# drprojects/DeepViewAgg

Hardware: AMD Instinct MI355X
Metric: points/sec fused fwd+bwd (1M pts, 32 views) (higher is better)
Workload: dtype bf16

## Files before the change

### deepviewagg_amd/csrc/chain_bwd.hip

```cpp
#include "chain_common.h"

namespace dva {
namespace chain {

struct ChainKeep {
  f32x16 z5, z6, t6;
  bf16x8 a2[2], a5[2], a6[2];
};
template <int W6F, int L6, bool MASK = true>
__device__ __forceinline__ void chain_forward(const uint4* s_ops, int lane, const float (*tabs)[TAB_FLOATS], int h,
                                              uint32_t keep, const float4& x, const f32x16& uacc, ChainKeep& k) {
  const f32x16 zero = {0};
  bf16x8 a1[2];
  asm volatile("" ::: "memory");
  const f32x16 t1 = CH_MFMA(lds_op(s_ops, OP_W1, lane), pack_x(x), bias_acc(tabs[0], T_B6, h));
  act_fold<MASK>(t1, keep, a1);
  const f32x16 t2 = mm32_lds(s_ops, OP_W2, lane, a1, bias_acc(tabs[1], T_B6, h));
  act_fold<MASK>(t2, keep, k.a2);
  k.z5 = mm32_lds(s_ops, OP_W5, lane, k.a2, uacc);
  act_pack<MASK>(k.z5, tabs[2], h, keep, k.a5);
  k.z6 = mm32_lds(s_ops, OP_W6, lane, k.a5, zero);
  if (L6 >= 1) k.t6 = mm32_lds(s_ops, W6F, lane, k.a5, bias_acc(tabs[3], T_B6, h));
  if (L6 >= 2) act_fold<MASK>(k.t6, keep, k.a6);
}
// ... 321 lines not shown
    const float* __restrict__ bn1, const float* __restrict__ bn2, const float* __restrict__ bn5,
    const float* __restrict__ bn6, const float* __restrict__ dc, double* __restrict__ stats6,
    float* __restrict__ dWs, float* __restrict__ dbs, int G, int64_t V, int64_t N, const float* __restrict__ qp,
    float qscale) {
  constexpr int L_W6F = 7, L_WST = 9, NOPS = KEYS ? 11 : 10;
  __shared__ __attribute__((aligned(16))) float s_tab[4][TAB_FLOATS];
  __shared__ __attribute__((aligned(16))) uint4 s_ops[NOPS * 64];
  __shared__ __attribute__((aligned(16))) bf16_t s_tc[4][32 * TSB], s_td[4][(KEYS ? 32 : 5) * TSB];
  float* s_red = reinterpret_cast<float*>(&s_tc[0][0]);
  static_assert(sizeof(bf16_t) * 4 * 32 * TSB >= sizeof(float) * D * D, "epilogue buffer");
  const int lane = threadIdx.x & 63, wv = threadIdx.x >> 6, j = lane & 31, h = lane >> 5;
  for (int i = threadIdx.x; i < 4 * (KEYS ? 32 : 5) * TSB; i += blockDim.x) (&s_td[0][0])[i] = 0;
  for (int i = threadIdx.x; i < 4 * 64; i += blockDim.x) s_ops[OP_W5 * 64 + i] = ops[OP_W5 * 64 + i];
  for (int i = threadIdx.x; i < (KEYS ? 128 : 64); i += blockDim.x)
    s_ops[L_WST * 64 + i] = ops[(KEYS ? OP_WKT : OP_WST) * 64 + i];
  fold_ops(s_ops, OP_W1, ops, OP_W1, 1, bn1);
  fold_ops(s_ops, OP_W2, ops, OP_W2, 2, bn2);
  fold_ops(s_ops, L_W6F, ops, OP_W6, 2, bn6);
  stage_tab(s_tab[0], bn1, nullptr);
  stage_tab(s_tab[1], bn2, nullptr);
  stage_tab(s_tab[2], bn5, nullptr);
  stage_tab(s_tab[3], bn6, nullptr);
  __syncthreads();
  const __amdgpu_buffer_rsrc_t X = make_rsrc(x_map, (uint64_t)V * 32), P = make_rsrc(vp, (uint64_t)V * 4),
                               U = make_rsrc(u, (uint64_t)N * 128), DC = make_rsrc(dc, (uint64_t)V * 16),
                               QP = make_rsrc(qp, KEYS ? (uint64_t)N * 128 : 0);
  bf16_t* tc = s_tc[wv];
  bf16_t* td = s_td[wv];
  f32x16 accS = {0};
  float dbsum[4] = {0.f, 0.f, 0.f, 0.f};
  float st[2][16];
#pragma unroll
  for (int r = 0; r < 16; ++r) st[0][r] = st[1][r] = 0.f;
  const int n_tiles = n_tiles_dev[0];
  int ta, tb;
  wave_tile_range(tiles, n_tiles, ta, tb);
  struct Pre {
    TileInfo ti;
    float4 x, dc;
    int vpj;
  };
  run_tiles<Pre>(tiles, ta, tb, [&](const TileInfo& ti, int t) {
    Pre p;
    p.ti = ti;
    const bool ok = j < p.ti.nv;
    const uint32_t view = (uint32_t)(p.ti.v0 + j);
    p.x = as_f4(ld128(X, ok ? view * 32u + 16u * h : OOB));
    p.vpj = (int)ld32(P, ok ? view * 4u : OOB);
    p.dc = as_f4(ld128(DC, ok && (KEYS || h == 0) ? view * 16u : OOB));
    return p;
  }, [&](const Pre& p) {
    const bool ok = j < p.ti.nv;
    const uint32_t keep = ok ? 0xffffffffu : 0u;
    const f32x16 uacc = load_u(U, ok, p.vpj, h);
    ChainKeep k;
    chain_forward<L_W6F, 2, false>(s_ops, lane, s_tab, h, keep, p.x, uacc, k);
    if constexpr (KEYS) {
      bf16x8 dkp[2];
      dkeys_operand(p.dc, QP, ok, p.vpj, h, G, qscale, dkp);
      tileN_put_packed(tc, j, h, k.a6);
      tileN_put_packed(td, j, h, dkp);
      const f32x16 zero = {0};
      f32x16 dy6 = mm32_lds(s_ops, L_WST, lane, dkp, zero);
      dleaky_mul(k.t6, dy6);
      bn_bwd_stats(k.z6, dy6, st);
      wave_sync();
      accS = wgradN(td, tc, lane, accS);
      col_sum1(td, lane, dbsum[0]);
      wave_sync();
      return;
    }
    const float dc4[4] = {p.dc.x, p.dc.y, p.dc.z, p.dc.w};
    tileN_put_packed(tc, j, h, k.a6);
    if (h == 0) {
      const uint32_t d01 = pack_bf16x2(dc4[0], dc4[1]), d23 = pack_bf16x2(dc4[2], dc4[3]);
      td[0 * TSB + j] = (bf16_t)(d01 & 0xffffu);
      td[1 * TSB + j] = (bf16_t)(d01 >> 16);
      td[2 * TSB + j] = (bf16_t)(d23 & 0xffffu);
      td[3 * TSB + j] = (bf16_t)(d23 >> 16);
#pragma unroll
      for (int g = 0; g < 4; ++g) dbsum[g] += dc4[g];
    }
    f32x16 dy6 = score_bwd<L_WST>(s_ops, lane, dc4, h);
    dleaky_mul(k.t6, dy6);
    bn_bwd_stats(k.z6, dy6, st);
    wave_sync();
    accS = wgradN_T(tc, td, lane, j, 4, h, accS);
    wave_sync();
  });
  if constexpr (KEYS) {
    flush_matrix_nat(accS, dWs, D, D, false, s_red, true);
    flush_stats<2>(st, stats6, s_red);
    __syncthreads();
    {
      uint32_t a = __float_as_uint(dbsum[0]), b = a;
      swap_halves(a, b);
      const float tot = dbsum[0] + __uint_as_float((threadIdx.x & 32) ? a : b);
      if (h == 0) s_red[wv * 32 + j] = tot;
    }
    __syncthreads();
    if (threadIdx.x < 32)
      atomicAdd(&dbs[cperm(threadIdx.x)], (s_red[threadIdx.x] + s_red[32 + threadIdx.x]) +
                                             (s_red[64 + threadIdx.x] + s_red[96 + threadIdx.x]));
    return;
  }
  flush_matrix_nat(accS, dWs, D, G, true, s_red, false);
  flush_stats<2>(st, stats6, s_red);
  __syncthreads();
#pragma unroll
  for (int g = 0; g < 4; ++g) {
    float v = dbsum[g];
#pragma unroll
    for (int off = 1; off < 64; off <<= 1) v += __shfl_xor(v, off);
    if (lane == 0) s_red[wv * 4 + g] = v;
  }
  __syncthreads();
  if ((int)threadIdx.x < G) atomicAdd(&dbs[threadIdx.x], (s_red[threadIdx.x] + s_red[4 + threadIdx.x]) +
                                                           (s_red[8 + threadIdx.x] + s_red[12 + threadIdx.x]));
}

template <typename A16>
__device__ __forceinline__ void store_da(__amdgpu_buffer_rsrc_t R, bool ok, uint32_t view, int h, const A16& da) {
  float t[16];
#pragma unroll
  for (int r = 0; r < 16; ++r) t[r] = da[r];
  const bf16x8 lo = pack8(&t[0]), hi = pack8(&t[8]);
  const uint32_t off = ok ? view * 64u + 32u * h : OOB;
  st128(R, off, __builtin_bit_cast(u32x4, lo));
  st128(R, ok ? off + 16u : OOB, __builtin_bit_cast(u32x4, hi));
}
__device__ __forceinline__ f32x16 unpack_da(const u32x4& lo, const u32x4& hi) {
  const uint32_t w[8] = {lo.x, lo.y, lo.z, lo.w, hi.x, hi.y, hi.z, hi.w};
  f32x16 d;
#pragma unroll
  for (int i = 0; i < 8; ++i) {
    d[2 * i] = __uint_as_float(w[i] << 16);
    d[2 * i + 1] = __uint_as_float(w[i] & 0xffff0000u);
  }
  return d;
}

template <int STAGE, int OCC, bool KEYS = false>
__global__ __launch_bounds__(256, OCC) void layer_bwd_kernel(
    const float* __restrict__ x_map, const int32_t* __restrict__ vp, const float* __restrict__ u,
    const int2* __restrict__ tiles, const int32_t* __restrict__ n_tiles_dev, const uint4* __restrict__ ops,
    const float* __restrict__ bn1, const float* __restrict__ bn2, const float* __restrict__ bn5,
    const float* __restrict__ bn6, const float* __restrict__ sm2, const float* __restrict__ sm5,
    const float* __restrict__ sm6, const float* __restrict__ dc, const int32_t* __restrict__ arg,
    const float* __restrict__ dpooled, const bf16_t* __restrict__ da_in, bf16_t* __restrict__ da_out,
    float* __restrict__ dW,
    float* __restrict__ du, float* __restrict__ Pm, double* __restrict__ stats, int G, int64_t V, int64_t N,
    const float* __restrict__ qp, float qscale) {
  __shared__ __attribute__((aligned(16))) float s_tab[4][TAB_FLOATS];
  __shared__ __attribute__((aligned(16))) bf16_t s_ta[4][32 * TSB], s_tb[4][32 * TSB];
  constexpr int TD_ROWS = 17;
  __shared__ __attribute__((aligned(16))) bf16_t s_tc[STAGE == 2 ? 4 : 1][STAGE == 2 ? 32 * TSB : 8], s_td[STAGE == 2 ? 4 : 1][STAGE == 2 ? (TD_ROWS + 1) * TSB : 8];
  __shared__ __attribute__((aligned(16))) bf16_t s_ind[STAGE == 5 ? 4 : 1][STAGE == 5 ? 32 * TSB : 8];
  __shared__ int s_plp[STAGE == 5 ? 4 : 1][32];
  static_assert(sizeof(bf16_t) * 4 * 32 * TSB >= sizeof(float) * D * D, "epilogue buffer");
  float* s_red = reinterpret_cast<float*>(&s_ta[0][0]);
  constexpr int NOPS = STAGE == 6 ? (KEYS ? 13 : 12) : (STAGE == 5 ? 9 : 6);
  constexpr int L_W5T = 5, L_W2T = 3, L_W2F = 7, L_W1F = 5, L6_W6T = 7, L6_WST = 9, L6_W6F = KEYS ? 11 : 10;
  __shared__ __attribute__((aligned(16))) uint4 s_ops[NOPS * 64];
  const int lane = threadIdx.x & 63, wv = threadIdx.x >> 6, j = lane & 31, h = lane >> 5;
  if (STAGE == 6) {
    for (int i = threadIdx.x; i < 5 * 64; i += blockDim.x) {
      const int blk = i >> 6, l = i & 63;
      if (blk < 2) s_ops[(OP_W5 + blk) * 64 + l] = ops[(OP_W5 + blk) * 64 + l];
      else if (blk < 4) s_ops[(OP_W6 + blk - 2) * 64 + l] = ops[(OP_W6 + blk - 2) * 64 + l];
      else if (!KEYS) s_ops[L6_WST * 64 + l] = ops[OP_WST * 64 + l];
    }
    if (KEYS) {
      for (int i = threadIdx.x; i < 2 * 64; i += blockDim.x) s_ops[L6_WST * 64 + i] = ops[OP_WKT * 64 + i];
    }
    for (int i = threadIdx.x; i < 2 * 64; i += blockDim.x) s_ops[L6_W6T * 64 + i] = ops[OP_W6T * 64 + i];
    fold_ops(s_ops, OP_W1, ops, OP_W1, 1, bn1);
    fold_ops(s_ops, OP_W2, ops, OP_W2, 2, bn2);
    fold_ops(s_ops, L6_W6F, ops, OP_W6, 2, bn6);
  } else {
    for (int i = threadIdx.x; i < (STAGE == 5 ? 7 : 5) * 64; i += blockDim.x) {
      int op = i >> 6;
      if (STAGE == 5 && op >= 5) op = OP_W5T + (op - 5);
      if (STAGE == 2 && op >= 3) op = OP_W2T + (op - 3);
      s_ops[i] = ops[op * 64 + (i & 63)];
    }
    __syncthreads();
    if (STAGE == 5) {
      fold_ops(s_ops, OP_W1, ops, OP_W1, 1, bn1);
      fold_ops(s_ops, L_W2F, ops, OP_W2, 2, bn2);
    } else {
      fold_ops(s_ops, L_W1F, ops, OP_W1, 1, bn1);
    }
  }
  stage_tab(s_tab[0], bn1, nullptr);
  stage_tab(s_tab[1], bn2, STAGE == 2 ? sm2 : nullptr);
  stage_tab(s_tab[2], bn5, STAGE == 5 ? sm5 : nullptr);
  stage_tab(s_tab[3], bn6, STAGE == 6 ? sm6 : nullptr);
  for (int i = threadIdx.x; i < 4 * 32 * TSB; i += blockDim.x) {
    if (STAGE == 2) {
      if (i < 4 * (TD_ROWS + 1) * TSB) (&s_td[0][0])[i] = 0;
    } else if (STAGE == 5) {
      (&s_ind[0][0])[i] = 0;
    }
  }
  __syncthreads();
  const __amdgpu_buffer_rsrc_t X = make_rsrc(x_map, (uint64_t)V * 32), P = make_rsrc(vp, (uint64_t)V * 4),
                               U = make_rsrc(u, (uint64_t)N * 128), DC = make_rsrc(dc, (uint64_t)V * 16), QP = make_rsrc(qp, KEYS ? (uint64_t)N * 128 : 0),
                               AR = make_rsrc(arg, (uint64_t)N * 128), DP = make_rsrc(dpooled, (uint64_t)N * 128),
                               DI = make_rsrc(da_in, (uint64_t)V * 64), DO = make_rsrc(da_out, (uint64_t)V * 64);
  float st[2][16];
#pragma unroll
  for (int r = 0; r < 16; ++r) st[0][r] = st[1][r] = 0.f;
  f32x16 accW = {0}, accS = {0};
  bf16_t* ta = s_ta[wv];
  bf16_t* tb_ = s_tb[wv];
  bf16_t* tc = s_tc[STAGE == 2 ? wv : 0];
  bf16_t* td = s_td[STAGE == 2 ? wv : 0];
  bf16_t* ind = s_ind[STAGE == 5 ? wv : 0];
  int* plp = s_plp[STAGE == 5 ? wv : 0];

  const int n_tiles = n_tiles_dev[0];
  int t0, t1;
  wave_tile_range(tiles, n_tiles, t0, t1);
  struct Pre {
    TileInfo ti;
    float4 x, dc;
    u32x4 dlo, dhi;
    int vpj;
  };
  run_tiles<Pre>(tiles, t0, t1, [&](const TileInfo& ti, int t) {
    Pre p;
    p.ti = ti;
    const bool ok = j < p.ti.nv;
    const uint32_t view = (uint32_t)(p.ti.v0 + j);
    p.x = as_f4(ld128(X, ok ? view * 32u + 16u * h : OOB));
    p.vpj = (int)ld32(P, ok ? view * 4u : OOB);
    if (STAGE == 2) {
      p.dlo = ld128(DI, ok ? view * 64u + 32u * h : OOB);
      p.dhi = ld128(DI, ok ? view * 64u + 32u * h + 16u : OOB);
    }
    return p;
  }, [&](const Pre& p) {
    const int nv = p.ti.nv;
    const bool ok = j < nv;
    const uint32_t keep = ok ? 0xffffffffu : 0u;
    const uint32_t view = (uint32_t)(p.ti.v0 + j);
    const f32x16 zero = {0};
    float dz[16];
    bf16x8 dzp[2];
    if constexpr (STAGE == 6) {
      const f32x16 uacc = load_u(U, ok, p.vpj, h);
      const float4 dcv = as_f4(ld128(DC, ok && (KEYS || h == 0) ? view * 16u : OOB));
      bf16x8 a5[2];
      f32x16 z5;
      {
        bf16x8 a1[2], a2[2];
        asm volatile("" ::: "memory");
        const f32x16 t1 = CH_MFMA(lds_op(s_ops, OP_W1, lane), pack_x(p.x), bias_acc(s_tab[0], T_B6, h));
        act_fold<false>(t1, keep, a1);
        const f32x16 t2 = mm32_lds(s_ops, OP_W2, lane, a1, bias_acc(s_tab[1], T_B6, h));
        act_fold<false>(t2, keep, a2);
        z5 = mm32_lds(s_ops, OP_W5, lane, a2, uacc);
        act_pack<false>(z5, s_tab[2], h, keep, a5);
      }
      tileN_put_packed(tb_, j, h, a5);
      const float dc4[4] = {dcv.x, dcv.y, dcv.z, dcv.w};
      {
        f32x16 dy6;
        if constexpr (KEYS) {
          bf16x8 dkp[2];
          dkeys_operand(dcv, QP, ok, p.vpj, h, G, qscale, dkp);
          dy6 = mm32_lds(s_ops, L6_WST, lane, dkp, zero);
        } else {
          dy6 = score_bwd<L6_WST>(s_ops, lane, dc4, h);
        }
        {
          const f32x16 t6 = mm32_lds(s_ops, L6_W6F, lane, a5, bias_acc(s_tab[3], T_B6, h));
          dleaky_mul(t6, dy6);
        }
        const f32x16 z6 = mm32_lds(s_ops, OP_W6, lane, a5, zero);
        bn_bwd_apply(z6, dy6, s_tab[3], h, dz);
      }
      pack16(dz, keep, dzp);
      tileN_put_packed(ta, j, h, dzp);
      const f32x16 da5 = mm32_lds(s_ops, L6_W6T, lane, dzp, zero);
      layer_bwd<true, false>(z5, da5, s_tab[2], h, ok, st, dz);
      store_da(DO, ok, view, h, dz);
      wave_sync();
      accW = wgradN(ta, tb_, lane, accW);
      wave_sync();
    } else if constexpr (STAGE == 5) {
      f32x16 uacc = load_u(U, ok, p.vpj, h);
      const u32x4 dlo = ld128(DI, ok ? view * 64u + 32u * h : OOB);
      const u32x4 dhi = ld128(DI, ok ? view * 64u + 32u * h + 16u : OOB);
      bf16x8 a1[2], a2[2];
      asm volatile("" ::: "memory");
      const f32x16 t1 = CH_MFMA(lds_op(s_ops, OP_W1, lane), pack_x(p.x), bias_acc(s_tab[0], T_B6, h));
      act_fold(t1, 0xffffffffu, a1);
      {
        const f32x16 t2 = mm32_lds(s_ops, L_W2F, lane, a1, bias_acc(s_tab[1], T_B6, h));
        act_fold<false>(t2, keep, a2);
      }
      {
        const f32x16 z5 = mm32_lds(s_ops, OP_W5, lane, a2, uacc);
        const f32x16 dy5 = unpack_da(dlo, dhi);
        bn_bwd_apply(z5, dy5, s_tab[2], h, dz);
      }
      pack16(dz, keep, dzp);
      tileN_put_packed(ta, j, h, dzp);
      tileN_put_packed(tb_, j, h, a2);
      const int prv = shfl(p.vpj, lane - 1);
      const bool is_start = ok && (j == 0 || prv != p.vpj);
      const uint32_t smask = (uint32_t)__ballot(is_start);
      const int lpj = __popc(smask & (0xffffffffu >> (31 - j))) - 1;
      const int nseg = __popc(smask);
      if (h == 0 && ok) {
        ind[lpj * TSB + j] = (bf16_t)0x3f80;
        if (is_start) plp[lpj] = p.vpj;
      }
      f32x16 dy2 = mm32_lds(s_ops, L_W5T, lane, dzp, zero);
      {
        const f32x16 t2 = mm32_lds(s_ops, L_W2F, lane, a1, bias_acc(s_tab[1], T_B6, h));
        dleaky_mul(t2, dy2);
      }
      store_da(DO, ok, view, h, dy2);
      {
        const f32x16 z2 = mm32_lds(s_ops, OP_W2, lane, a1, zero);
        bn_bwd_stats(z2, dy2, st);
      }
      wave_sync();
      accW = wgradN(ta, tb_, lane, accW);
      const int frag = p.ti.frag;
      const f32x16 accU = wgradN_T(ta, ind, lane, j, 32, h, zero);
      if (h == 0 && ok) ind[lpj * TSB + j] = 0;
      {
        const bool wr = j < nseg;
        const uint32_t pt = wr ? (uint32_t)plp[j] : 0u;
        if (frag == 0) {
          const __amdgpu_buffer_rsrc_t DU = make_rsrc(du, (uint64_t)N * 128);
#pragma unroll
          for (int qq = 0; qq < 4; ++qq)
            st128(DU, wr ? pt * 128u + (uint32_t)(4 * (qq >> 1) + 8 * h + 16 * (qq & 1)) * 4u : OOB,
                  as_u4(accU[4 * qq], accU[4 * qq + 1], accU[4 * qq + 2], accU[4 * qq + 3]));
        } else if (wr) {
#pragma unroll
          for (int r = 0; r < 16; ++r) atomicAdd(&du[(size_t)pt * D + cperm(chan(r, h))], accU[r]);
        }
      }
      wave_sync();
    } else {
      u32x4 arq[4], dpq[4];
#pragma unroll
      for (int qq = 0; qq < 4; ++qq) {
        const uint32_t off = ok ? (uint32_t)p.vpj * 128u + (8u * qq + 4u * h) * 4u : OOB;
        arq[qq] = ld128(AR, off);
        dpq[qq] = ld128(DP, off);
      }
      bf16x8 a1[2];
      asm volatile("" ::: "memory");
      const bf16x8 xp = pack_x(p.x);
      {
        const f32x16 t1 = CH_MFMA(lds_op(s_ops, L_W1F, lane), xp, bias_acc(s_tab[0], T_B6, h));
        act_fold<false>(t1, keep, a1);
      }
      f32x16 da2t = unpack_da(p.dlo, p.dhi);
      {
        const int vg = p.ti.v0 + j;
#pragma unroll
        for (int qq = 0; qq < 4; ++qq) {
          const uint32_t ai[4] = {arq[qq].x, arq[qq].y, arq[qq].z, arq[qq].w};
          const uint32_t di[4] = {dpq[qq].x, dpq[qq].y, dpq[qq].z, dpq[qq].w};
#pragma unroll
          for (int e = 0; e < 4; ++e)
            da2t[4 * qq + e] += (int)ai[e] == vg ? __uint_as_float(di[e]) : 0.f;
        }
      }
      asm volatile("" ::: "memory");
      {
        const f32x16 z2 = mm32_lds(s_ops, OP_W2, lane, a1, zero);
        bn_bwd_apply(z2, da2t, s_tab[1], h, dz);
      }
      pack16(dz, keep, dzp);
      tileN_put_packed(ta, j, h, dzp);
      tileN_put_packed(tb_, j, h, a1);
      const f32x16 da1 = mm32_lds(s_ops, L_W2T, lane, dzp, zero);
      {
        const f32x16 t1 = CH_MFMA(lds_op(s_ops, L_W1F, lane), xp, bias_acc(s_tab[0], T_B6, h));
#pragma unroll
        for (int r = 0; r < 16; ++r) dz[r] = da1[r] * dleaky(t1[r]);
      }
      {
        bf16x8 dy1p[2];
        pack16(dz, 0xffffffffu, dy1p);
        tileN_put_packed(tc, j, h, dy1p);
      }
      {
        const float xs[4] = {p.x.x, p.x.y, p.x.z, p.x.w};
#pragma unroll
        for (int e = 0; e < 4; e += 2) {
          const uint32_t hi2 = pack_bf16x2(xs[e], xs[e + 1]);
          tileT_put(td, 4 * h + e, 4 * h + e + 1, j, xs[e], xs[e + 1]);
          tileT_put(td, 8 + 4 * h + e, 8 + 4 * h + e + 1, j, xs[e] - __uint_as_float(hi2 << 16),
                    xs[e + 1] - __uint_as_float(hi2 & 0xffff0000u));
        }
        if (h == 0) td[16 * TSB + j] = ok ? (bf16_t)0x3f80 : (bf16_t)0;
      }
      wave_sync();
      accW = wgradN(ta, tb_, lane, accW);
      accS = wgradN_T(tc, td, lane, j, TD_ROWS, h, accS);
      wave_sync();
    }
  });
  flush_matrix_nat(accW, dW, STAGE == 5 ? 2 * D : D, D, false, s_red, true);
  if (STAGE == 2) flush_matrix_nat(accS, Pm, 20, 17, false, s_red, false);
  else flush_stats<2>(st, stats, s_red);
}

__global__ __launch_bounds__(256) void route_stats_kernel(const float* __restrict__ zstar,
                                                          const float* __restrict__ dpooled,
                                                          const float* __restrict__ bn2,
                                                          const int64_t* __restrict__ ptr, double* __restrict__ stats,
                                                          float* __restrict__ dpy, int64_t N) {
  __shared__ float s_red[2 * D];
  const int q = threadIdx.x & 7, sub = threadIdx.x >> 3;
  float g[4], b[4], iv[4], mm[4], s1[4], s2[4];
#pragma unroll
  for (int e = 0; e < 4; ++e) {
    const int c = 4 * q + e;
    g[e] = bn2[2 * D + c] * bn2[D + c];
    b[e] = bn2[3 * D + c] - bn2[c] * g[e];
    iv[e] = bn2[D + c];
    mm[e] = -bn2[c] * bn2[D + c];
    s1[e] = s2[e] = 0.f;
  }
  const int64_t stride = (int64_t)gridDim.x * 32;
  for (int64_t p0 = (int64_t)blockIdx.x * 32 + sub; p0 < N; p0 += 2 * stride) {
    const int64_t p1 = p0 + stride;
    const bool ok0 = ptr[p0 + 1] > ptr[p0], ok1 = p1 < N && ptr[p1 + 1] > ptr[p1];
    float4 z0 = make_float4(0.f, 0.f, 0.f, 0.f), d0 = z0, z1 = z0, d1 = z0;
    if (ok0) {
      z0 = *reinterpret_cast<const float4*>(zstar + p0 * D + 4 * q);
      d0 = *reinterpret_cast<const float4*>(dpooled + p0 * D + 4 * q);
    }
    if (ok1) {
      z1 = *reinterpret_cast<const float4*>(zstar + p1 * D + 4 * q);
      d1 = *reinterpret_cast<const float4*>(dpooled + p1 * D + 4 * q);
    }
    const float zz[2][4] = {{z0.x, z0.y, z0.z, z0.w}, {z1.x, z1.y, z1.z, z1.w}};
    const float dd[2][4] = {{d0.x, d0.y, d0.z, d0.w}, {d1.x, d1.y, d1.z, d1.w}};
    float dyv[2][4];
#pragma unroll
    for (int u = 0; u < 2; ++u) {
#pragma unroll
      for (int e = 0; e < 4; ++e) {
        const float dy = dd[u][e] * dleaky(__builtin_fmaf(zz[u][e], g[e], b[e]));
        dyv[u][e] = dy;
        s1[e] += dy;
        s2[e] = __builtin_fmaf(dy, __builtin_fmaf(zz[u][e], iv[e], mm[e]), s2[e]);
      }
    }
    *reinterpret_cast<float4*>(dpy + p0 * D + 4 * q) = make_float4(dyv[0][0], dyv[0][1], dyv[0][2], dyv[0][3]);
    if (p1 < N) *reinterpret_cast<float4*>(dpy + p1 * D + 4 * q) = make_float4(dyv[1][0], dyv[1][1], dyv[1][2], dyv[1][3]);
  }
  if (threadIdx.x < 2 * D) s_red[threadIdx.x] = 0.f;
  __syncthreads();
#pragma unroll
  for (int e = 0; e < 4; ++e) {
    for (int off = 8; off < 64; off <<= 1) {
      s1[e] += __shfl_xor(s1[e], off);
      s2[e] += __shfl_xor(s2[e], off);
    }
    if ((threadIdx.x & 63) < 8) {
      atomicAdd(&s_red[4 * q + e], s1[e]);
      atomicAdd(&s_red[D + 4 * q + e], s2[e]);
    }
  }
  __syncthreads();
  if (threadIdx.x < 2 * D) atomicAdd(&stats[threadIdx.x], (double)s_red[threadIdx.x]);
}

__global__ void bn_bwd_consts_kernel(double* __restrict__ stats, const float* __restrict__ bn, double inv_m,
                                     int do_hat, float* __restrict__ sm, float* __restrict__ dgamma,
                                     float* __restrict__ dbeta, int C) {
  for (int c = threadIdx.x; c < C; c += blockDim.x) {
    const double s1 = stats[c];
    double s2 = stats[C + c];
    if (do_hat) {
      s2 = (double)bn[C + c] * (s2 - (double)bn[c] * s1);
      stats[C + c] = s2;
    }
    if (sm) {
      sm[c] = (float)(s1 * inv_m);
      sm[C + c] = (float)(s2 * inv_m);
    }
    if (dgamma) dgamma[c] = (float)s2;
    if (dbeta) dbeta[c] = (float)s1;
  }
}

__global__ void dw1_kernel(const float* __restrict__ P, const double* __restrict__ mom, const float* __restrict__ W1,
                           int exact_w1, const float* __restrict__ bn1, const float* __restrict__ sm1,
                           float* __restrict__ dW1) {
  const int i = threadIdx.x >> 3, k = threadIdx.x & 7;
  double acc = 0.0;
#pragma unroll
  for (int l = 0; l < 8; ++l) {
    const int a = l < k ? l : k, b = l < k ? k : l;
    const double xx = mom[8 + a * 8 - a * (a - 1) / 2 + (b - a)];
    acc += (exact_w1 ? (double)W1[i * 8 + l] : (double)bf2f(f2bf(W1[i * 8 + l]))) * xx;
  }
  const double mean = bn1[i], inv = bn1[D + i], gam = bn1[2 * D + i], sx = mom[k];
  const double q = inv * (acc - mean * sx);
  const double pik = (double)P[i * 20 + k] + (double)P[i * 20 + 8 + k];
  dW1[i * 8 + k] = (float)(gam * inv * (pik - (double)sm1[i] * sx - (double)sm1[D + i] * q));
}

__global__ void stats1_from_p_kernel(const float* __restrict__ P, const float* __restrict__ W1, int exact_w1,
                                     double* __restrict__ stats) {
  const int n = threadIdx.x;
  if (n >= D) return;
  double s2 = 0.0;
#pragma unroll
  for (int f = 0; f < 8; ++f)
    s2 += (exact_w1 ? (double)W1[n * 8 + f] : (double)bf2f(f2bf(W1[n * 8 + f]))) *
          ((double)P[n * 20 + f] + (double)P[n * 20 + 8 + f]);
  stats[n] = (double)P[n * 20 + 16];
  stats[D + n] = s2;
}

}
}

using namespace dva;
using namespace dva::chain;

// ... 235 lines not shown
```

### deepviewagg_amd/csrc/chain_common.h

```cpp
#pragma once
#include <cstdlib>
#include "dva_common.h"

namespace dva {
namespace chain {

typedef float f32x16 __attribute__((ext_vector_type(16)));
typedef __bf16 bf16x8 __attribute__((ext_vector_type(8)));
typedef uint32_t u32x4 __attribute__((ext_vector_type(4)));
typedef uint32_t u32x2 __attribute__((ext_vector_type(2)));

#define CH_MFMA(a, b, c) __builtin_amdgcn_mfma_f32_32x32x16_bf16((a), (b), (c), 0, 0, 0)

constexpr int D = 32;
constexpr float SLOPE = 0.2f;
constexpr uint32_t OOB = 0x7ffffff0u;

__host__ __device__ __forceinline__ int chan(int r, int h) { return (r & 3) + 8 * (r >> 2) + 4 * h; }

enum {
  OP_W1 = 0,
  OP_W2 = 1,
  OP_W5 = 3,
  OP_W6 = 5,
// ... 251 lines not shown
constexpr int N_OPS32 = 7;
constexpr int OPS_UINT4 = N_OPS * 64 + N_OPS32 * 64 * 2;
__device__ __forceinline__ void fold_ops(uint4* s_ops, int dst, const uint4* __restrict__ ops, int op, int n_blocks,
                                         const float* __restrict__ bn) {
  const float4* w32 = reinterpret_cast<const float4*>(ops + N_OPS * 64);
  for (int i = threadIdx.x; i < n_blocks * 64; i += blockDim.x) {
    const int n = i & 31;
    const float s = 0.6f * bn[2 * D + n] * bn[D + n];
    const float4 a = w32[(op * 64 + i) * 2], b = w32[(op * 64 + i) * 2 + 1];
    s_ops[dst * 64 + i] = make_uint4(pack_bf16x2(a.x * s, a.y * s), pack_bf16x2(a.z * s, a.w * s),
                                     pack_bf16x2(b.x * s, b.y * s), pack_bf16x2(b.z * s, b.w * s));
  }
}
__device__ __forceinline__ bf16x8 load_op_fold(const uint4* __restrict__ ops, int op, int lane,
                                               const float* __restrict__ bn) {
  const float4* w32 = reinterpret_cast<const float4*>(ops + N_OPS * 64) + (op * 64 + lane) * 2;
  const int n = lane & 31;
  const float s = 0.6f * bn[2 * D + n] * bn[D + n];
  const float4 a = w32[0], b = w32[1];
  const u32x4 v = {pack_bf16x2(a.x * s, a.y * s), pack_bf16x2(a.z * s, a.w * s), pack_bf16x2(b.x * s, b.y * s),
                   pack_bf16x2(b.z * s, b.w * s)};
  return __builtin_bit_cast(bf16x8, v);
}
__device__ __forceinline__ WOp load_wop_fold(const uint4* __restrict__ ops, int op, int lane,
                                             const float* __restrict__ bn) {
  WOp w;
  w.m[0] = load_op_fold(ops, op, lane, bn);
  w.m[1] = load_op_fold(ops, op + 1, lane, bn);
  return w;
}
__device__ __forceinline__ f32x16 bias_acc(const float* tab, int row, int h) {
  asm volatile("" ::: "memory");
  float b[16];
  tab16(tab, row, h, b);
  f32x16 c;
#pragma unroll
  for (int r = 0; r < 16; ++r) c[r] = b[r];
  return c;
}
template <bool MASK = true>
__device__ __forceinline__ void act_fold(const f32x16& t, uint32_t keep, bf16x8 (&a)[2], float* sum = nullptr) {
  float av[16];
#pragma unroll
  for (int r = 0; r < 16; ++r) av[r] = __builtin_fmaf(__builtin_fabsf(t[r]), 0.6666667f, t[r]);
  if (sum && keep) {
#pragma unroll
    for (int r = 0; r < 16; ++r) sum[r] += av[r];
  }
  a[0] = MASK ? mask8(pack8(&av[0]), keep) : pack8(&av[0]);
  a[1] = MASK ? mask8(pack8(&av[8]), keep) : pack8(&av[8]);
}

constexpr int STATS_RED_FLOATS = 4 * 3 * D;
template <int NV>
__device__ __forceinline__ void flush_stats(float (&st)[NV][16], double* __restrict__ out, float* s_red) {
  const int lane = threadIdx.x & 63, h = lane >> 5, wv = threadIdx.x >> 6;
  __syncthreads();
#pragma unroll
  for (int n = 0; n < NV; ++n) {
#pragma unroll
    for (int r = 0; r < 16; ++r) {
      float v = st[n][r];
#pragma unroll
      for (int off = 1; off < 32; off <<= 1) v += __shfl_xor(v, off);
      if ((lane & 31) == 0) s_red[wv * (NV * D) + n * D + chan(r, h)] = v;
    }
  }
  __syncthreads();
  const int n_waves = blockDim.x >> 6;
  for (int i = threadIdx.x; i < NV * D; i += blockDim.x) {
    double acc = 0.0;
    for (int w = 0; w < n_waves; ++w) acc += (double)s_red[w * (NV * D) + i];
    atomicAdd(&out[i], acc);
  }
}

constexpr int TSB = 40;
__device__ __forceinline__ void tileT_put(bf16_t* tile, int c0, int c1, int v, float x0, float x1) {
  const uint32_t d = pack_bf16x2(x0, x1);
  tile[c0 * TSB + v] = (bf16_t)(d & 0xffffu);
  tile[c1 * TSB + v] = (bf16_t)(d >> 16);
}
__device__ __forceinline__ void tileT_put_acc(bf16_t* tile, int v, int h, const float* x) {
#pragma unroll
  for (int r = 0; r < 16; r += 2) tileT_put(tile, chan(r, h), chan(r + 1, h), v, x[r], x[r + 1]);
}
__device__ __forceinline__ bf16x8 tileT_get(const bf16_t* tile, int c, int h, int m) {
  return *reinterpret_cast<const bf16x8*>(tile + c * TSB + 16 * m + 8 * h);
}

template <bool STATS, bool APPLY>
__device__ __forceinline__ void layer_bwd(const f32x16& z, const f32x16& da, const float* tab, int h, bool ok,
                                          float (&st)[2][16], float (&dz)[16]) {
  asm volatile("" ::: "memory");
#pragma unroll
  for (int q = 0; q < 4; ++q) {
    const int o = 16 * h + 4 * q;
    const float4 g4 = *reinterpret_cast<const float4*>(tab + T_G * D + o);
    const float4 b4 = *reinterpret_cast<const float4*>(tab + T_B * D + o);
    const float g[4] = {g4.x, g4.y, g4.z, g4.w}, b[4] = {b4.x, b4.y, b4.z, b4.w};
    float k1[4] = {0.f, 0.f, 0.f, 0.f}, k2[4] = {0.f, 0.f, 0.f, 0.f};
    if (APPLY) {
      const float4 a4 = *reinterpret_cast<const float4*>(tab + T_K1 * D + o);
      const float4 c4 = *reinterpret_cast<const float4*>(tab + T_K2 * D + o);
      k1[0] = a4.x; k1[1] = a4.y; k1[2] = a4.z; k1[3] = a4.w;
      k2[0] = c4.x; k2[1] = c4.y; k2[2] = c4.z; k2[3] = c4.w;
    }
#pragma unroll
    for (int e = 0; e < 4; ++e) {
      const int r = 4 * q + e;
      const float y = __builtin_fmaf(z[r], g[e], b[e]);
      const float dy = y > 0.f ? da[r] : SLOPE * da[r];
      if (STATS) {
        st[0][r] += dy;
        st[1][r] = __builtin_fmaf(dy, z[r], st[1][r]);
      }
      if (APPLY) dz[r] = __builtin_fmaf(-k2[e], z[r], __builtin_fmaf(g[e], dy, -k1[e]));
      else dz[r] = dy;
    }
  }
}
__device__ __forceinline__ void dleaky_mul(const f32x16& t, f32x16& da) {
#pragma unroll
  for (int r = 0; r < 16; ++r) da[r] = t[r] > 0.f ? da[r] : SLOPE * da[r];
}
__device__ __forceinline__ void bn_bwd_stats(const f32x16& z, const f32x16& dy, float (&st)[2][16]) {
#pragma unroll
  for (int r = 0; r < 16; ++r) {
    st[0][r] += dy[r];
    st[1][r] = __builtin_fmaf(dy[r], z[r], st[1][r]);
  }
}
__device__ __forceinline__ void bn_bwd_apply(const f32x16& z, const f32x16& dy, const float* tab, int h,
                                             float (&dz)[16]) {
  asm volatile("" ::: "memory");
#pragma unroll
  for (int q = 0; q < 4; ++q) {
    const int o = 16 * h + 4 * q;
    const float4 g4 = *reinterpret_cast<const float4*>(tab + T_G * D + o);
    const float4 a4 = *reinterpret_cast<const float4*>(tab + T_K1 * D + o);
    const float4 c4 = *reinterpret_cast<const float4*>(tab + T_K2 * D + o);
    const float g[4] = {g4.x, g4.y, g4.z, g4.w}, k1[4] = {a4.x, a4.y, a4.z, a4.w}, k2[4] = {c4.x, c4.y, c4.z, c4.w};
#pragma unroll
    for (int e = 0; e < 4; ++e) {
      const int r = 4 * q + e;
      dz[r] = __builtin_fmaf(-k2[e], z[r], __builtin_fmaf(g[e], dy[r], -k1[e]));
    }
  }
}
__device__ __forceinline__ void pack16(const float (&x)[16], uint32_t keep, bf16x8 (&a)[2]) {
  a[0] = mask8(pack8(&x[0]), keep);
  a[1] = mask8(pack8(&x[8]), keep);
}
__device__ __forceinline__ void tileT_put_packed(bf16_t* tile, int v, int h, const bf16x8 (&a)[2]) {
#pragma unroll
  for (int m = 0; m < 2; ++m) {
    const u32x4 w = __builtin_bit_cast(u32x4, a[m]);
    const uint32_t ww[4] = {w.x, w.y, w.z, w.w};
#pragma unroll
    for (int i = 0; i < 4; ++i) {
      tile[chan(8 * m + 2 * i, h) * TSB + v] = (bf16_t)(ww[i] & 0xffffu);
      tile[chan(8 * m + 2 * i + 1, h) * TSB + v] = (bf16_t)(ww[i] >> 16);
    }
  }
}
__device__ __forceinline__ f32x16 wgrad(const bf16_t* ta, const bf16_t* tb, int j, int h, f32x16 acc) {
  acc = CH_MFMA(tileT_get(ta, j, h, 0), tileT_get(tb, j, h, 0), acc);
  acc = CH_MFMA(tileT_get(ta, j, h, 1), tileT_get(tb, j, h, 1), acc);
  return acc;
}
__device__ __forceinline__ f32x16 wgrad_short(const bf16_t* ta, const bf16_t* tb, int j, int jb_max, int h,
                                              f32x16 acc) {
  const int jb = j < jb_max ? j : jb_max;
  acc = CH_MFMA(tileT_get(ta, j, h, 0), tileT_get(tb, jb, h, 0), acc);
  acc = CH_MFMA(tileT_get(ta, j, h, 1), tileT_get(tb, jb, h, 1), acc);
  return acc;
}
typedef short s16x4 __attribute__((ext_vector_type(4)));
__device__ __forceinline__ int cperm(int n) { return chan(n & 15, n >> 4); }
__device__ __forceinline__ void tileN_put_packed(bf16_t* tile, int v, int h, const bf16x8 (&a)[2]) {
  *reinterpret_cast<bf16x8*>(tile + v * TSB + 16 * h) = a[0];
  *reinterpret_cast<bf16x8*>(tile + v * TSB + 16 * h + 8) = a[1];
}
__device__ __forceinline__ bf16x8 tileN_get(const bf16_t* tile, int lane, int m) {
  typedef __attribute__((address_space(3))) s16x4* lds_s16x4;
  const int ip = lane & 15, g = lane >> 4;
  const bf16_t* base = tile + (16 * m + 8 * (g >> 1) + (ip >> 2)) * TSB + 16 * (g & 1) + 4 * (ip & 3);
  const s16x4 lo = __builtin_amdgcn_ds_read_tr16_b64_v4i16((lds_s16x4)base);
  const s16x4 hi = __builtin_amdgcn_ds_read_tr16_b64_v4i16((lds_s16x4)(base + 4 * TSB));
  const u32x2 l2 = __builtin_bit_cast(u32x2, lo), h2 = __builtin_bit_cast(u32x2, hi);
  const u32x4 v = {l2.x, l2.y, h2.x, h2.y};
  return __builtin_bit_cast(bf16x8, v);
}
__device__ __forceinline__ f32x16 wgradN(const bf16_t* ta, const bf16_t* tb, int lane, f32x16 acc) {
  acc = CH_MFMA(tileN_get(ta, lane, 0), tileN_get(tb, lane, 0), acc);
  acc = CH_MFMA(tileN_get(ta, lane, 1), tileN_get(tb, lane, 1), acc);
  return acc;
}
__device__ __forceinline__ void unpack8(const bf16x8& v, float (&f)[8]) {
  const u32x4 u = __builtin_bit_cast(u32x4, v);
  const uint32_t w[4] = {u.x, u.y, u.z, u.w};
#pragma unroll
  for (int i = 0; i < 4; ++i) {
    f[2 * i] = __uint_as_float(w[i] << 16);
    f[2 * i + 1] = __uint_as_float(w[i] & 0xffff0000u);
  }
}
__device__ __forceinline__ void col_sum1(const bf16_t* tx, int lane, float& s) {
#pragma unroll
  for (int m = 0; m < 2; ++m) {
    float x[8];
    unpack8(tileN_get(tx, lane, m), x);
#pragma unroll
    for (int i = 0; i < 8; ++i) s += x[i];
  }
}
__device__ __forceinline__ f32x16 wgradN_T(const bf16_t* ta, const bf16_t* tb, int lane, int j, int jb_max, int h,
                                           f32x16 acc) {
  const int jb = j < jb_max ? j : jb_max;
  acc = CH_MFMA(tileN_get(ta, lane, 0), tileT_get(tb, jb, h, 0), acc);
  acc = CH_MFMA(tileN_get(ta, lane, 1), tileT_get(tb, jb, h, 1), acc);
  return acc;
}
__device__ __forceinline__ void flush_red(float* __restrict__ out, int ld, int ncol, bool transpose,
                                          const float* s_red) {
  for (int i = threadIdx.x; i < ncol * D; i += blockDim.x) {
    const int row = transpose ? i % D : i / ncol, col = transpose ? i / D : i % ncol;
    atomicAdd(&out[transpose ? col * ld + row : row * ld + col], s_red[row * D + col]);
  }
}

__device__ __forceinline__ void flush_matrix_nat(const f32x16& acc, float* __restrict__ out, int ld, int ncol,
                                                 bool transpose, float* s_red, bool cols_nat) {
  const int lane = threadIdx.x & 63, j = lane & 31, h = lane >> 5;
  __syncthreads();
  for (int i = threadIdx.x; i < D * D; i += blockDim.x) s_red[i] = 0.f;
  __syncthreads();
  if (j < ncol) {
    const int col = cols_nat ? cperm(j) : j;
#pragma unroll
    for (int r = 0; r < 16; ++r) atomicAdd(&s_red[cperm(chan(r, h)) * D + col], acc[r]);
  }
  __syncthreads();
  flush_red(out, ld, ncol, transpose, s_red);
}

__device__ __forceinline__ void flush_matrix(const f32x16& acc, float* __restrict__ out, int ld, int ncol,
                                             bool transpose, float* s_red) {
  const int lane = threadIdx.x & 63, j = lane & 31, h = lane >> 5;
  __syncthreads();
  for (int i = threadIdx.x; i < D * D; i += blockDim.x) s_red[i] = 0.f;
  __syncthreads();
  if (j < ncol) {
#pragma unroll
    for (int r = 0; r < 16; ++r) atomicAdd(&s_red[chan(r, h) * D + j], acc[r]);
  }
  __syncthreads();
  flush_red(out, ld, ncol, transpose, s_red);
}


static inline int chain_grid(int blocks_per_cu) {
  static int cus = 0;
  if (cus == 0) {
    int dev = 0;
    (void)hipGetDevice(&dev);
    (void)hipDeviceGetAttribute(&cus, hipDeviceAttributeMultiprocessorCount, dev);
    if (cus <= 0) cus = 256;
  }
  return cus * blocks_per_cu;
}

}
}

namespace dva {
namespace chain {

struct SegInfo {
  bool valid;
  bool pd[4];
  bool pb;
  int ss, se;
  uint32_t smask;
  uint32_t emask;
  int nseg;
};

template <int CTRL, int ROW_MASK = 0xf>
__device__ __forceinline__ int dpp_keep(int old, int x) {
  return __builtin_amdgcn_update_dpp(old, x, CTRL, ROW_MASK, 0xf, false);
}

__device__ __forceinline__ SegInfo seg_setup(int vpj, int j, int lane, int nv) {
  SegInfo s;
  s.valid = j < nv;
  const int lp = s.valid ? vpj : -1 - j;
  const int prv = dpp_keep<0x138>(lp, lp);
  const int nxt = dpp_keep<0x130>(lp, lp);
  const bool is_start = (j == 0) || (prv != lp);
  const bool is_end = (j == 31) || (nxt != lp);
  s.smask = (uint32_t)__ballot(is_start && s.valid);
  s.emask = (uint32_t)__ballot(is_end && s.valid);
  const uint32_t below = s.smask & (0xffffffffu >> (31 - j));
  s.ss = s.valid ? 31 - __clz((int)below) : j;
  s.se = s.valid ? j + (__ffs((int)(s.emask >> j)) - 1) : j;
// ... 89 lines not shown
```

Before: 104.8 million.

## Route pooled-argmax gradients per point via LDS and skip full-tile masking

In the stage-2 backward, when a tile's views cover only a few distinct points, the code now loads those points' argmax and pooled-gradient rows once with scalar-lane loads and scatters matching entries into an LDS routing tile. This replaces each lane loading full 128-byte argmax and gradient rows per view and comparing them. Per-wave shared tiles are merged into one contiguous buffer so the routing tile can alias existing space. Masking in pack16 is skipped when the tile is full. The change adds a wave-uniform branch, an extra wave sync, and LDS traffic on the per-point path.

```diff
diff --git a/deepviewagg_amd/csrc/chain_bwd.hip b/deepviewagg_amd/csrc/chain_bwd.hip
--- a/deepviewagg_amd/csrc/chain_bwd.hip
+++ b/deepviewagg_amd/csrc/chain_bwd.hip
@@ -497,13 +497,15 @@
     float* __restrict__ du, float* __restrict__ Pm, double* __restrict__ stats, int G, int64_t V, int64_t N,
     const float* __restrict__ qp, float qscale) {
   __shared__ __attribute__((aligned(16))) float s_tab[4][TAB_FLOATS];
-  __shared__ __attribute__((aligned(16))) bf16_t s_ta[4][32 * TSB], s_tb[4][32 * TSB];
   constexpr int TD_ROWS = 17;
-  __shared__ __attribute__((aligned(16))) bf16_t s_tc[STAGE == 2 ? 4 : 1][STAGE == 2 ? 32 * TSB : 8], s_td[STAGE == 2 ? 4 : 1][STAGE == 2 ? (TD_ROWS + 1) * TSB : 8];
+  constexpr int TILE_E = 32 * TSB, TD_E = (TD_ROWS + 1) * TSB, WAVE_E = STAGE == 2 ? 3 * TILE_E + TD_E : 2 * TILE_E;
+  constexpr int ROUTE_K = 2, ROUTE_LD = 36;
+  static_assert(sizeof(float) * 32 * ROUTE_LD <= sizeof(bf16_t) * 2 * TILE_E && ROUTE_K % 2 == 0, "routing tile");
+  __shared__ __attribute__((aligned(16))) bf16_t s_tiles[4][WAVE_E];
   __shared__ __attribute__((aligned(16))) bf16_t s_ind[STAGE == 5 ? 4 : 1][STAGE == 5 ? 32 * TSB : 8];
   __shared__ int s_plp[STAGE == 5 ? 4 : 1][32];
-  static_assert(sizeof(bf16_t) * 4 * 32 * TSB >= sizeof(float) * D * D, "epilogue buffer");
-  float* s_red = reinterpret_cast<float*>(&s_ta[0][0]);
+  static_assert(sizeof(bf16_t) * 4 * WAVE_E >= sizeof(float) * D * D, "epilogue buffer");
+  float* s_red = reinterpret_cast<float*>(&s_tiles[0][0]);
   constexpr int NOPS = STAGE == 6 ? (KEYS ? 13 : 12) : (STAGE == 5 ? 9 : 6);
   constexpr int L_W5T = 5, L_W2T = 3, L_W2F = 7, L_W1F = 5, L6_W6T = 7, L6_WST = 9, L6_W6F = KEYS ? 11 : 10;
   __shared__ __attribute__((aligned(16))) uint4 s_ops[NOPS * 64];
@@ -543,7 +545,7 @@
   stage_tab(s_tab[3], bn6, STAGE == 6 ? sm6 : nullptr);
   for (int i = threadIdx.x; i < 4 * 32 * TSB; i += blockDim.x) {
     if (STAGE == 2) {
-      if (i < 4 * (TD_ROWS + 1) * TSB) (&s_td[0][0])[i] = 0;
+      if (i < 4 * TD_E) s_tiles[i / TD_E][WAVE_E - TD_E + i % TD_E] = 0;
     } else if (STAGE == 5) {
       (&s_ind[0][0])[i] = 0;
     }
@@ -557,10 +559,10 @@
 #pragma unroll
   for (int r = 0; r < 16; ++r) st[0][r] = st[1][r] = 0.f;
   f32x16 accW = {0}, accS = {0};
-  bf16_t* ta = s_ta[wv];
-  bf16_t* tb_ = s_tb[wv];
-  bf16_t* tc = s_tc[STAGE == 2 ? wv : 0];
-  bf16_t* td = s_td[STAGE == 2 ? wv : 0];
+  bf16_t* ta = s_tiles[wv];
+  bf16_t* tb_ = ta + TILE_E;
+  bf16_t* tc = ta + 2 * TILE_E;
+  bf16_t* td = ta + (WAVE_E - TD_E);
   bf16_t* ind = s_ind[STAGE == 5 ? wv : 0];
   int* plp = s_plp[STAGE == 5 ? wv : 0];
 
@@ -626,7 +628,7 @@
         const f32x16 z6 = mm32_lds(s_ops, OP_W6, lane, a5, zero);
         bn_bwd_apply(z6, dy6, s_tab[3], h, dz);
       }
-      pack16(dz, keep, dzp);
+      pack16_tile(dz, nv, keep, dzp);
       tileN_put_packed(ta, j, h, dzp);
       const f32x16 da5 = mm32_lds(s_ops, L6_W6T, lane, dzp, zero);
       layer_bwd<true, false>(z5, da5, s_tab[2], h, ok, st, dz);
@@ -651,7 +653,7 @@
         const f32x16 dy5 = unpack_da(dlo, dhi);
         bn_bwd_apply(z5, dy5, s_tab[2], h, dz);
       }
-      pack16(dz, keep, dzp);
+      pack16_tile(dz, nv, keep, dzp);
       tileN_put_packed(ta, j, h, dzp);
       tileN_put_packed(tb_, j, h, a2);
       const int prv = shfl(p.vpj, lane - 1);
@@ -694,12 +696,38 @@
       }
       wave_sync();
     } else {
+      const int prv = shfl(p.vpj, lane - 1);
+      const uint32_t smask = (uint32_t)__ballot(ok && (j == 0 || prv != p.vpj));
+      const bool per_point = __popc(smask) <= ROUTE_K;
+      float* rt = reinterpret_cast<float*>(ta);
       u32x4 arq[4], dpq[4];
-#pragma unroll
-      for (int qq = 0; qq < 4; ++qq) {
-        const uint32_t off = ok ? (uint32_t)p.vpj * 128u + (8u * qq + 4u * h) * 4u : OOB;
-        arq[qq] = ld128(AR, off);
-        dpq[qq] = ld128(DP, off);
+      uint32_t rar[ROUTE_K / 2], rdp[ROUTE_K / 2];
+      bool rok[ROUTE_K / 2];
+      if (per_point) {
+        uint32_t m = smask;
+#pragma unroll
+        for (int i = 0; i < ROUTE_K / 2; ++i) {
+          const bool e0 = m != 0;
+          const int pt0 = __builtin_amdgcn_readlane(p.vpj, e0 ? __builtin_ctz(m) : 0);
+          m &= m - 1;
+          const bool e1 = m != 0;
+          const int pt1 = __builtin_amdgcn_readlane(p.vpj, e1 ? __builtin_ctz(m) : 0);
+          m &= m - 1;
+          rok[i] = h ? e1 : e0;
+          const uint32_t off = rok[i] ? (uint32_t)(h ? pt1 : pt0) * 128u + 4u * j : OOB;
+          rar[i] = ld32(AR, off);
+          rdp[i] = ld32(DP, off);
+        }
+        const float4 z4 = make_float4(0.f, 0.f, 0.f, 0.f);
+#pragma unroll
+        for (int qq = 0; qq < 4; ++qq) *reinterpret_cast<float4*>(rt + j * ROUTE_LD + 16 * h + 4 * qq) = z4;
+      } else {
+#pragma unroll
+        for (int qq = 0; qq < 4; ++qq) {
+          const uint32_t off = ok ? (uint32_t)p.vpj * 128u + (8u * qq + 4u * h) * 4u : OOB;
+          arq[qq] = ld128(AR, off);
+          dpq[qq] = ld128(DP, off);
+        }
       }
       bf16x8 a1[2];
       asm volatile("" ::: "memory");
@@ -709,7 +737,22 @@
         act_fold<false>(t1, keep, a1);
       }
       f32x16 da2t = unpack_da(p.dlo, p.dhi);
-      {
+      if (per_point) {
+#pragma unroll
+        for (int i = 0; i < ROUTE_K / 2; ++i) {
+          const uint32_t row = rar[i] - (uint32_t)p.ti.v0;
+          if (rok[i] && row < (uint32_t)nv) rt[row * ROUTE_LD + j] = __uint_as_float(rdp[i]);
+        }
+        wave_sync();
+#pragma unroll
+        for (int qq = 0; qq < 4; ++qq) {
+          const float4 r4 = *reinterpret_cast<const float4*>(rt + j * ROUTE_LD + 8 * qq + 4 * h);
+          da2t[4 * qq] += r4.x;
+          da2t[4 * qq + 1] += r4.y;
+          da2t[4 * qq + 2] += r4.z;
+          da2t[4 * qq + 3] += r4.w;
+        }
+      } else {
         const int vg = p.ti.v0 + j;
 #pragma unroll
         for (int qq = 0; qq < 4; ++qq) {
@@ -725,7 +768,7 @@
         const f32x16 z2 = mm32_lds(s_ops, OP_W2, lane, a1, zero);
         bn_bwd_apply(z2, da2t, s_tab[1], h, dz);
       }
-      pack16(dz, keep, dzp);
+      pack16_tile(dz, nv, keep, dzp);
       tileN_put_packed(ta, j, h, dzp);
       tileN_put_packed(tb_, j, h, a1);
       const f32x16 da1 = mm32_lds(s_ops, L_W2T, lane, dzp, zero);
diff --git a/deepviewagg_amd/csrc/chain_common.h b/deepviewagg_amd/csrc/chain_common.h
--- a/deepviewagg_amd/csrc/chain_common.h
+++ b/deepviewagg_amd/csrc/chain_common.h
@@ -427,6 +427,15 @@
   a[0] = mask8(pack8(&x[0]), keep);
   a[1] = mask8(pack8(&x[8]), keep);
 }
+__device__ __forceinline__ void pack16_tile(const float (&x)[16], int nv, uint32_t keep, bf16x8 (&a)[2]) {
+  a[0] = pack8(&x[0]);
+  a[1] = pack8(&x[8]);
+  if (nv < 32) {
+    asm volatile("");
+    a[0] = mask8(a[0], keep);
+    a[1] = mask8(a[1], keep);
+  }
+}
 __device__ __forceinline__ void tileT_put_packed(bf16_t* tile, int v, int h, const bf16x8 (&a)[2]) {
 #pragma unroll
   for (int m = 0; m < 2; ++m) {
```

Result: no change. 103.8 million (-0.9%).
